# microscopic-image-analysis/DiffPointRasterisation.jl

Measured on AMD Instinct MI355X. Metric: M points/s fwd+bwd, 10M pts→256³ grid; HBM GB/s vs roofline, higher is better.
Workload: dtype f32

## Files before the change

### diffpointrasterisation.jl_amd/csrc/dpr_tiled.hip

```cpp
#include <hip/hip_runtime.h>

#include <cstring>
#include <mutex>
#include <set>
#include <type_traits>
#include <utility>

#include "dpr_tiled_impl.h"

namespace dpr {

template <int NO>
__device__ __forceinline__ int primary_tile(const int (&ref0)[NO], const TileGeom<NO>& tg) {
    int t = 0, stride = 1;
    bool in = true;
#pragma unroll
    for (int d = 0; d < NO; ++d) {
        const int r = ref0[d] < 0 ? 0 : ref0[d];
        int c = r / TileDims<NO>::T[d];
        if (d == NO - 1) {
            c -= tg.tz0;
            in = (unsigned)c < (unsigned)tg.nt[d];
        }
        t += c * stride;
// ... 1133 lines not shown
        return;
    }
    char* const wsp = ws + (size_t)blockIdx.y * pose_stride;
    const RunDesc* __restrict__ desc = (const RunDesc*)(wsp + off_desc);
    const uint32_t* __restrict__ blk_ndesc = (const uint32_t*)(wsp + off_bdesc);
    const uint32_t* __restrict__ tile_dstart = (const uint32_t*)(wsp + off_dstart);
    uint32_t* __restrict__ tile_cursor = (uint32_t*)(wsp + off_dcursor);
    RunDesc* __restrict__ sorted = (RunDesc*)(wsp + off_sdesc);
    const int lane = threadIdx.x & (kWave - 1), wave = threadIdx.x / kWave;
    if (fused) {
        const uint32_t* __restrict__ tile_ndesc = (const uint32_t*)(wsp + ra.off_ltot);
        const int NT = ra.NT;
        uint32_t c[4], sum = 0;
#pragma unroll
        for (int q = 0; q < 4; ++q) {
            const int i = threadIdx.x * 4 + q;
            c[q] = i < NT ? tile_ndesc[i] : 0u;
            sum += c[q];
        }
        uint32_t incl = sum;
#pragma unroll
        for (int o = 1; o < kWave; o <<= 1) {
            const uint32_t v = __shfl_up(incl, o, kWave);
            if (lane >= o) incl += v;
        }
        if (lane == kWave - 1) wsum[wave] = incl;
        __syncthreads();
        uint32_t run = incl - sum;
        for (int wv = 0; wv < wave; ++wv) run += wsum[wv];
#pragma unroll
        for (int q = 0; q < 4; ++q) {
            const int i = threadIdx.x * 4 + q;
            if (i < NT) s_dstart[i] = run;
            run += c[q];
        }
        __syncthreads();
    }
    const unsigned nblocks = fused ? gridDim.x - 1 : gridDim.x;
    const int64_t wave0 = (int64_t)blockIdx.x * (1024 / kWave) + wave;
    const int64_t nwaves = (int64_t)nblocks * (1024 / kWave);
    for (int64_t sub = wave0; sub < nsub; sub += nwaves) {
        const uint32_t n = blk_ndesc[sub] < (uint32_t)S ? blk_ndesc[sub] : (uint32_t)S;
        for (uint32_t i = lane; i < n; i += kWave) {
            const RunDesc d = desc[(size_t)sub * S + i];
            const uint32_t base = fused ? s_dstart[d.tile()] : tile_dstart[d.tile()];
            sorted[base + atomicAdd(&tile_cursor[d.tile()], 1u)] = d;
        }
    }
}

template <bool FIX, typename T, int NI, int NO, bool HAS_PW, typename R>
__device__ __forceinline__ void splat_record(const R& rc, bool active, const Pose<T, NI, NO>& ps,
                                             const GridDesc<NO>& gd, const int (&x0)[NO],
                                             double* __restrict__ acc, const FixScale& fs) {
    T pt[NI];
#pragma unroll
    for (int j = 0; j < NI; ++j) pt[j] = rc.v[j];
    const T w = HAS_PW ? ps.ow * rc.v[HAS_PW ? 3 : 0] : ps.ow * T(1);
    int ref0[NO];
    T dlo[NO];
    ref_and_deltas<T, NI, NO>(pt, ps, gd, ref0, dlo);
    int lb[NO];
    bool low_ok[NO];
#pragma unroll
    for (int d = 0; d < NO; ++d) {
        lb[d] = ref0[d] - x0[d];
        lb[d] = lb[d] < -1 ? -1 : (lb[d] > TileDims<NO>::T[d] - 1 ? TileDims<NO>::T[d] - 1 : lb[d]);
        low_ok[d] = lb[d] >= 0;
    }
    bool interior = true;
#pragma unroll
    for (int d = 0; d < NO; ++d) interior = interior && low_ok[d];
    if (active && interior) {
        double* base = &acc[lds_index<NO>(lb)];
#pragma unroll
        for (int s = 0; s < (1 << NO); ++s)
            cell_add<FIX, T>(base + nbr_lds_offset<NO>(s), voxel_weight<T, NO>(dlo, s, w), fs);
    } else if (active) {
#pragma unroll
        for (int s = 0; s < (1 << NO); ++s) {
            int l[NO];
            bool ok = true;
#pragma unroll
            for (int d = 0; d < NO; ++d) {
                const int sd = (s >> d) & 1;
                ok = ok && (sd || low_ok[d]);
                l[d] = (sd || low_ok[d]) ? lb[d] + sd : 0;
            }
            const T v = voxel_weight<T, NO>(dlo, s, w);
            cell_add<FIX, T>(&acc[lds_index<NO>(l)], ok ? v : T(0), fs);
        }
    }
}

template <bool FIX, typename T, int NI, int NO, typename R>
__device__ __forceinline__ void splat_record_jvp(const R& rc, const Rec4<T>& cf, bool active,
                                                 const Pose<T, NI, NO>& ps, const GridDesc<NO>& gd,
                                                 const int (&x0)[NO], double* __restrict__ acc, const FixScale& fs) {
    T pt[NI];
#pragma unroll
    for (int j = 0; j < NI; ++j) pt[j] = rc.v[j];
    int ref0[NO];
    T dlo[NO];
    ref_and_deltas<T, NI, NO>(pt, ps, gd, ref0, dlo);
    T bc[NO];
#pragma unroll
    for (int n = 0; n < NO; ++n) bc[n] = cf.v[1 + n];
    int lb[NO];
    bool low_ok[NO];
#pragma unroll
    for (int d = 0; d < NO; ++d) {
        lb[d] = ref0[d] - x0[d];
        lb[d] = lb[d] < -1 ? -1 : (lb[d] > TileDims<NO>::T[d] - 1 ? TileDims<NO>::T[d] - 1 : lb[d]);
        low_ok[d] = lb[d] >= 0;
    }
    bool interior = true;
#pragma unroll
    for (int d = 0; d < NO; ++d) interior = interior && low_ok[d];
    if (active && interior) {
        double* base = &acc[lds_index<NO>(lb)];
#pragma unroll
        for (int s = 0; s < (1 << NO); ++s)
            cell_add<FIX, T>(base + nbr_lds_offset<NO>(s), jvp_deposit<T, NO>(cf.v[0], bc, dlo, s), fs);
    } else if (active) {
#pragma unroll
        for (int s = 0; s < (1 << NO); ++s) {
            int l[NO];
            bool ok = true;
#pragma unroll
            for (int d = 0; d < NO; ++d) {
                const int sd = (s >> d) & 1;
                ok = ok && (sd || low_ok[d]);
                l[d] = (sd || low_ok[d]) ? lb[d] + sd : 0;
            }
            const T v = jvp_deposit<T, NO>(cf.v[0], bc, dlo, s);
            cell_add<FIX, T>(&acc[lds_index<NO>(l)], ok ? v : T(0), fs);
        }
    }
}

template <typename T, int NO>
__device__ __forceinline__ void flush_tile(const double* __restrict__ acc, const FixScale& fs, double bgv,
                                           const GridDesc<NO>& gd, const int (&x0)[NO], bool ghost_tile,
                                           T* __restrict__ o, T* __restrict__ hb) {
    constexpr int NVH = tile_voxels_halo<NO>();
    constexpr int TX = TileDims<NO>::T[0], TY = TileDims<NO>::T[1];
    constexpr int TZ = (NO == 3) ? TileDims<NO>::T[NO - 1] : 0;
    constexpr int ROWS = NVH / (TX + 1);
    constexpr int RPW = kWave / TX;
    static_assert(kWave % TX == 0, "tile rows must divide the wavefront");
    constexpr int NW = kSplatThreads / kWave;
    constexpr int kFB = 4;
    const int lane = threadIdx.x & (kWave - 1);
    const int x = lane % TX;
    const bool x_ok = x0[0] + x < gd.n[0];
    for (int row0 = (threadIdx.x / kWave) * RPW; row0 < ROWS; row0 += NW * RPW * kFB) {
        double raw[kFB];
        int rows[kFB];
#pragma unroll
        for (int u = 0; u < kFB; ++u) {
            int row = row0 + u * NW * RPW + lane / TX;
            if (RPW == 1) row = __builtin_amdgcn_readfirstlane(row);
            rows[u] = row;
            raw[u] = acc[(row < ROWS ? row : 0) * (TX + 1) + x];
        }
#pragma unroll
        for (int u = 0; u < kFB; ++u) {
            const int row = rows[u];
            if (row >= ROWS) continue;
            const int l1 = row % (TY + 1), l2 = (NO == 3) ? row / (TY + 1) : 0;
            const double a = fix_value(raw[u], fs);
            const bool owned = l1 < TY && (NO == 2 || l2 < TZ);
            if (owned) {
                const int g1 = x0[1] + l1, g2 = (NO == 3) ? x0[NO - 1] + l2 : 0;
                const bool in = g1 < gd.n[1] && (NO == 2 || g2 < gd.n[NO - 1]);
                if (in && x_ok && !ghost_tile)
                    __builtin_nontemporal_store(
                        (T)(bgv + a),
                        &o[((NO == 3) ? (size_t)g2 * gd.n[1] + g1 : (size_t)g1) * gd.n[0] + x0[0] + x]);
            } else {
                int h[NO];
                h[0] = x;
                h[1] = l1;
                if (NO == 3) h[NO - 1] = l2;
                hb[halo_index<NO>(h)] = (T)a;
            }
        }
    }
    for (int row = threadIdx.x; row < ROWS; row += kSplatThreads)
        hb[row] = (T)fix_value(acc[row * (TX + 1) + TX], fs);
}

template <typename T, int NI, int NO, bool HAS_PW, bool W3, bool WPL = false, bool JVP = false>
__global__ __launch_bounds__(kSplatThreads) void k_tile_splat(
    GridDesc<NO> gd, TileGeom<NO> tg, const RecT<T, W3>* __restrict__ rec,
    const WorkItem* __restrict__ items, const uint32_t* __restrict__ n_items,
    const uint32_t* __restrict__ tile_slab, const T* __restrict__ rot,
    const T* __restrict__ trans, const T* __restrict__ ow, const T* __restrict__ bg, int64_t b0,
    T* __restrict__ out, T* __restrict__ halo, T* __restrict__ ovf, int blocked,
    const uint32_t* __restrict__ maxpw, int fixed, const T* __restrict__ wplane) {
    static_assert(!WPL || (HAS_PW && !W3), "weight planes go with 4-word records and point weights");
    static_assert(!JVP || (HAS_PW && !W3 && !WPL), "coefficient records go with 4-word records");
    constexpr int NVH = tile_voxels_halo<NO>();
    __shared__ double acc[NVH];
    const uint32_t n_it = *n_items;
    const uint32_t order_flag = n_items[1];
    const float maxw_call = sizeof(T) == 4 ? guarded_max_weight(1.f, maxpw, HAS_PW) : __builtin_inff();
    const WorkItem item = items[blockIdx.x];
    Pose<T, NI, NO> ps = load_pose<T, NI, NO>(rot, trans, ow, b0);
    for (int i = threadIdx.x; i < NVH; i += kSplatThreads) acc[i] = 0.0;
    if (blockIdx.x >= n_it) return;
    if (blocked == 2) blocked = (NI == NO) ? (int)order_flag : 0;
    const int tile = (int)(item.tile % (uint32_t)tg.NT);
    const int64_t b = b0 + (int64_t)(item.tile / (uint32_t)tg.NT);
    int x0[NO], tc[NO];
    tile_origin<NO>(tile, tg, x0, tc);
    if (b != b0) ps = load_pose<T, NI, NO>(rot, trans, ow, b);
    uint32_t r1 = item.end;
    uint32_t r = item.begin;
    uint32_t step = kSplatThreads;
    if (blocked) {
        const uint32_t per = (r1 - r + kSplatThreads - 1) / kSplatThreads;
        r += threadIdx.x * per;
        r1 = (r + per < r1) ? r + per : r1;
        step = 1;
    } else {
        r += threadIdx.x;
    }
    constexpr int kPF = 2;
    RecT<T, W3> nxt[kPF];
    T nxt_w[WPL ? kPF : 1];
    Rec4<T> nxt_c[JVP ? kPF : 1];
    const Rec4<T>* const coef = (const Rec4<T>*)wplane;
#pragma unroll
    for (int u = 0; u < kPF; ++u) {
        const uint32_t ru = r + u * step;
        const uint32_t rl = ru < r1 ? ru : (r1 > item.begin ? r1 - 1 : item.begin);
        nxt[u] = rec[rl];
        if constexpr (WPL) nxt_w[u] = wplane[rl];
        if constexpr (JVP) nxt_c[u] = coef[rl];
    }
    lds_barrier();
    const FixScale fs = fix_scale(sizeof(T) == 4 ? fabsf((float)ps.ow) * maxw_call : __builtin_inff(),
                                  item.end - item.begin, fixed);
    auto record_loop = [&](auto fix_tag) {
        constexpr bool FIX = decltype(fix_tag)::value;
        while (r < r1) {
            RecT<T, W3> cur[kPF];
#pragma unroll
            for (int u = 0; u < kPF; ++u) cur[u] = nxt[u];
            if constexpr (WPL) {
#pragma unroll
                for (int u = 0; u < kPF; ++u) cur[u].v[3] = nxt_w[u];
            }
            Rec4<T> cur_c[JVP ? kPF : 1];
            if constexpr (JVP) {
#pragma unroll
                for (int u = 0; u < kPF; ++u) cur_c[u] = nxt_c[u];
            }
            const uint32_t r_cur = r;
            r += kPF * step;
#pragma unroll
            for (int u = 0; u < kPF; ++u) {
                const uint32_t ru = r + u * step;
                nxt[u] = rec[ru < r1 ? ru : r1 - 1];
                if constexpr (WPL) nxt_w[u] = wplane[ru < r1 ? ru : r1 - 1];
                if constexpr (JVP) nxt_c[u] = coef[ru < r1 ? ru : r1 - 1];
            }
#pragma unroll
            for (int u = 0; u < kPF; ++u) {
                if constexpr (JVP)
                    splat_record_jvp<FIX, T, NI, NO>(cur[u], cur_c[u], r_cur + u * step < r1, ps, gd, x0, acc, fs);
                else
                    splat_record<FIX, T, NI, NO, HAS_PW>(cur[u], r_cur + u * step < r1, ps, gd, x0, acc, fs);
            }
        }
    };
    if (fs.mul != 0.0) record_loop(std::true_type{});
    else record_loop(std::false_type{});
    lds_barrier();
    if ((item.part_nparts >> 16) > 1) {
        T* slab = ovf + (size_t)(tile_slab[item.tile] + (item.part_nparts & 0xffffu)) * NVH;
        constexpr int kSB = 4;
        for (int i0 = threadIdx.x; i0 < NVH; i0 += kSplatThreads * kSB) {
            double raw[kSB];
#pragma unroll
            for (int u = 0; u < kSB; ++u) {
                const int i = i0 + u * kSplatThreads;
                raw[u] = acc[i < NVH ? i : NVH - 1];
            }
#pragma unroll
            for (int u = 0; u < kSB; ++u) {
                const int i = i0 + u * kSplatThreads;
                if (i < NVH) slab[i] = (T)fix_value(raw[u], fs);
            }
        }
        return;
    }
    const double bgv = bg ? (double)bg[b] : 0.0;
    flush_tile<T, NO>(acc, fs, bgv, gd, x0, tg.ghost && tc[NO - 1] == 0 ,
                      out + b * gd.G, halo + (size_t)item.tile * halo_count<NO>());
}

template <typename T, int NI, int NO, bool HAS_PW, bool W3, bool RUNS>
__global__ __launch_bounds__(kSplatThreads, kSplatRunsOcc) void k_tile_splat_runs(
    GridDesc<NO> gd, TileGeom<NO> tg, const RecT<T, W3>* __restrict__ rec,
    const RunDesc* __restrict__ runs, uint32_t max_rec,
    const WorkItem* __restrict__ items, const uint32_t* __restrict__ n_items,
    const uint32_t* __restrict__ tile_slab, const T* __restrict__ rot,
    const T* __restrict__ trans, const T* __restrict__ ow, const T* __restrict__ bg, int64_t b0,
    T* __restrict__ out, T* __restrict__ halo, T* __restrict__ ovf, int blocked,
    const uint32_t* __restrict__ maxpw, int fixed) {
    constexpr int NVH = tile_voxels_halo<NO>();
    __shared__ double acc[NVH];
    const uint32_t n_it = *n_items;
    const WorkItem item = items[blockIdx.x];
    const float maxw_call = sizeof(T) == 4 ? guarded_max_weight(1.f, maxpw, HAS_PW) : __builtin_inff();
    Pose<T, NI, NO> ps = load_pose<T, NI, NO>(rot, trans, ow, b0);
    for (int i = threadIdx.x; i < NVH; i += kSplatThreads) acc[i] = 0.0;
    if (blockIdx.x >= n_it) return;
    const int tile = (int)(item.tile % (uint32_t)tg.NT);
    const int64_t b = b0 + (int64_t)(item.tile / (uint32_t)tg.NT);
    int x0[NO], tc[NO];
    tile_origin<NO>(tile, tg, x0, tc);
    if (b != b0) ps = load_pose<T, NI, NO>(rot, trans, ow, b);
    constexpr int kPF = 2;
    uint32_t n_bound = (item.end - item.begin) < (1u << 19) ? (item.end - item.begin) * 4096u : max_rec;
    n_bound = n_bound < max_rec ? n_bound : max_rec;
    const FixScale fs = fix_scale(sizeof(T) == 4 ? fabsf((float)ps.ow) * maxw_call : __builtin_inff(), n_bound, fixed);
    {
        __shared__ RunTable<kMaxRuns> rt;
        for (uint32_t d0 = item.begin; d0 < item.end; d0 += kMaxRuns) {
            const uint32_t d1 = (d0 + kMaxRuns < item.end) ? d0 + kMaxRuns : item.end;
            const int nruns = (int)(d1 - d0);
            const uint32_t n = load_runs(rt, runs, d0, d1, max_rec);
            const uint32_t per = (n + kSplatThreads - 1) / kSplatThreads;
            const uint32_t step = blocked ? 1u : (uint32_t)kSplatThreads;
            uint32_t i = blocked ? threadIdx.x * per : threadIdx.x;
            const uint32_t i1 = blocked ? ((i + per < n) ? i + per : n) : n;
            if (i < i1) {
                RunCursor cu;
                cu.seek(rt, i, nruns);
                uint32_t fetched = i;
                RecT<T, W3> nxt[kPF];
#pragma unroll
                for (int u = 0; u < kPF; ++u) {
                    const bool adv = fetched + step < i1;
                    nxt[u] = rec[cu.next(rt, adv ? step : 0u, nruns, adv)];
                    fetched += adv ? step : 0u;
                }
                while (i < i1) {
                    RecT<T, W3> cur[kPF];
#pragma unroll
                    for (int u = 0; u < kPF; ++u) cur[u] = nxt[u];
                    const uint32_t i_cur = i;
                    i += kPF * step;
#pragma unroll
                    for (int u = 0; u < kPF; ++u) {
                        const bool adv = fetched + step < i1;
                        nxt[u] = rec[cu.next(rt, adv ? step : 0u, nruns, adv)];
                        fetched += adv ? step : 0u;
                    }
#pragma unroll
                    for (int u = 0; u < kPF; ++u) {
                        if (fs.mul != 0.0)
                            splat_record<true, T, NI, NO, HAS_PW>(cur[u], i_cur + u * step < i1, ps, gd, x0, acc, fs);
                        else
                            splat_record<false, T, NI, NO, HAS_PW>(cur[u], i_cur + u * step < i1, ps, gd, x0, acc, fs);
                    }
                }
            }
            __syncthreads();
        }
    }
    lds_barrier();
    if ((item.part_nparts >> 16) > 1) {
        T* slab = ovf + (size_t)(tile_slab[item.tile] + (item.part_nparts & 0xffffu)) * NVH;
        constexpr int kSB = 4;
        for (int i0 = threadIdx.x; i0 < NVH; i0 += kSplatThreads * kSB) {
            double raw[kSB];
#pragma unroll
            for (int u = 0; u < kSB; ++u) {
                const int i = i0 + u * kSplatThreads;
                raw[u] = acc[i < NVH ? i : NVH - 1];
            }
#pragma unroll
            for (int u = 0; u < kSB; ++u) {
                const int i = i0 + u * kSplatThreads;
                if (i < NVH) slab[i] = (T)fix_value(raw[u], fs);
            }
        }
        return;
    }
    const double bgv = bg ? (double)bg[b] : 0.0;
    flush_tile<T, NO>(acc, fs, bgv, gd, x0, tg.ghost && tc[NO - 1] == 0 ,
                      out + b * gd.G, halo + (size_t)item.tile * halo_count<NO>());
}

template <int NO> __host__ __device__ constexpr int low_face_count() {
    if (NO == 2) return TileDims<2>::T[0] + TileDims<2>::T[1] - 1;
    return TileDims<3>::T[0] * TileDims<3>::T[1] + TileDims<3>::T[0] * (TileDims<3>::T[2] - 1) +
           (TileDims<3>::T[1] - 1) * (TileDims<3>::T[2] - 1);
}
template <int NO> __device__ __forceinline__ void low_face_coords(int i, int (&l)[NO]) {
    constexpr int TX = TileDims<NO>::T[0], TY = TileDims<NO>::T[1];
    if constexpr (NO == 2) {
        if (i < TX) {
            l[0] = i;
            l[1] = 0;
        } else {
            l[0] = 0;
            l[1] = 1 + (i - TX);
        }
    } else {
        constexpr int TZ = TileDims<NO>::T[2];
        if (i < TX * TY) {
            l[0] = i % TX;
            l[1] = i / TX;
            l[2] = 0;
        } else if (i < TX * TY + TX * (TZ - 1)) {
            const int j = i - TX * TY;
            l[0] = j % TX;
            l[1] = 0;
            l[2] = 1 + j / TX;
        } else {
            const int j = i - TX * TY - TX * (TZ - 1);
            l[0] = 0;
            l[1] = 1 + j % (TY - 1);
            l[2] = 1 + j / (TY - 1);
        }
    }
}

template <typename T, int NO>
__device__ __forceinline__ void halo_gather_tile(const GridDesc<NO>& gd, const TileGeom<NO>& tg,
                                                 const T* __restrict__ halo,
                                                 const T* __restrict__ ovf,
                                                 const uint32_t* __restrict__ tile_parts,
                                                 const uint32_t* __restrict__ tile_slab,
                                                 const T* __restrict__ bg, int64_t b0,
                                                 T* __restrict__ out, bool any_split, int ptile,
                                                 bool split, int c) {
    constexpr int NV = tile_voxels<NO>();
    constexpr int NVH = tile_voxels_halo<NO>();
    constexpr int CH = kSplitChunks;
    const int i_begin = split ? c * 256 : 0;
    const int i_end = split ? NV : low_face_count<NO>();
    const int tile = ptile % tg.NT;
    const int pbase = ptile - tile;
    const int64_t b = b0 + ptile / tg.NT;
    const int i_step = split ? 256 * CH : 256;
    int x0[NO], tc[NO];
    tile_origin<NO>(tile, tg, x0, tc);
    if (tg.ghost && tc[NO - 1] == 0) return;
    T* o = out + b * gd.G;
    constexpr int NC = 1 << NO;
    uint32_t nparts[NC], nslab[NC];
    bool nvalid[NC], any_nbr_split = false;
    int nsrc[NC];
#pragma unroll
    for (int m = 1; m < NC; ++m) {
        bool v = true;
        int src = ptile, tstride = 1;
#pragma unroll
        for (int d = 0; d < NO; ++d) {
            if ((m >> d) & 1) {
                v = v && tc[d] > 0;
                src -= tstride;
            }
            tstride *= tg.nt[d];
        }
        nvalid[m] = v;
        nsrc[m] = v ? src : ptile;
        nparts[m] = any_split ? tile_parts[nsrc[m]] : 1u;
        nslab[m] = any_split ? tile_slab[nsrc[m]] : 0u;
        any_nbr_split = any_nbr_split || (v && nparts[m] > 1);
    }
    if constexpr (NO == 3 && TileDims<NO>::T[0] == kWave) {
        if (split) {
            constexpr int TX = TileDims<NO>::T[0], TY = TileDims<NO>::T[1], TZ = TileDims<NO>::T[2];
            constexpr int YF = (TY + 1) * (TZ + 1), ZF = YF + TX * (TZ + 1);
            constexpr int NW = 256 / kWave, RIT = kSplitRows / NW;
            static_assert(kSplitRows % NW == 0 && (TY * TZ) % kSplitRows == 0, "whole rows per wave");
            static_assert(kSplitChunks * kSplitRows == TY * TZ, "chunks cover the tile");
            const int lane = threadIdx.x & (kWave - 1), wave = threadIdx.x / kWave;
            const uint32_t my_parts = tile_parts[ptile], my_slab = tile_slab[ptile];
            const double bgv = bg ? (double)bg[b] : 0.0;
            const bool x_ok = x0[0] + lane < gd.n[0];
            const size_t HC = halo_count<NO>();
            double own[RIT];
            bool act[RIT];
            int offs[RIT], cell[RIT], l1s[RIT], l2s[RIT];
#pragma unroll
            for (int k = 0; k < RIT; ++k) {
                const int row = __builtin_amdgcn_readfirstlane(c * kSplitRows + wave * RIT + k);
                l1s[k] = row % TY;
                l2s[k] = row / TY;
                const int g1 = x0[1] + l1s[k], g2 = x0[2] + l2s[k];
                act[k] = x_ok && g1 < gd.n[1] && g2 < gd.n[2];
                offs[k] = act[k] ? (g2 * gd.n[1] + g1) * gd.n[0] + x0[0] + lane : 0;
                cell[k] = lane + (TX + 1) * (l1s[k] + (TY + 1) * l2s[k]);
                own[k] = bgv;
            }
            const T* sp = ovf + (size_t)my_slab * NVH;
            for (uint32_t q = 0; q < my_parts; ++q) {
                T a[RIT];
#pragma unroll
                for (int k = 0; k < RIT; ++k) a[k] = sp[(size_t)q * NVH + cell[k]];
#pragma unroll
                for (int k = 0; k < RIT; ++k) own[k] += (double)a[k];
            }
            auto nbr = [&](int m, bool on, int hidx, int ncell) -> double {
                if (nparts[m] > 1) {
                    const T* np_ = ovf + (size_t)nslab[m] * NVH + (on ? ncell : 0);
                    double sum = 0.0;
                    for (uint32_t q = 0; q < nparts[m]; ++q) sum += (double)np_[(size_t)q * NVH];
                    return on ? sum : 0.0;
                }
                const T v = halo[on ? (size_t)nsrc[m] * HC + hidx : (size_t)0];
                return on ? (double)v : 0.0;
            };
#pragma unroll
            for (int k = 0; k < RIT; ++k) {
                const int l1 = l1s[k], l2 = l2s[k];
                const bool lowy = l1 == 0, lowz = l2 == 0, l0z = lane == 0;
                if (!(lowy || lowz || nvalid[1])) {
                    if (act[k]) o[offs[k]] = (T)own[k];
                    continue;
                }
                double add = 0.0;
                if (nvalid[1]) add += nbr(1, act[k] && l0z, l1 + (TY + 1) * l2, TX + (TX + 1) * (l1 + (TY + 1) * l2));
                if (lowy && nvalid[2]) add += nbr(2, act[k], YF + lane + TX * l2, lane + (TX + 1) * (TY + (TY + 1) * l2));
                if (lowy && nvalid[3]) add += nbr(3, act[k] && l0z, TY + (TY + 1) * l2, TX + (TX + 1) * (TY + (TY + 1) * l2));
                if (lowz && nvalid[4]) add += nbr(4, act[k], ZF + lane + TX * l1, lane + (TX + 1) * (l1 + (TY + 1) * TZ));
                if (lowz && nvalid[5]) add += nbr(5, act[k] && l0z, l1 + (TY + 1) * TZ, TX + (TX + 1) * (l1 + (TY + 1) * TZ));
                if (lowy && lowz && nvalid[6])
                    add += nbr(6, act[k], YF + TX * TZ + lane, lane + (TX + 1) * (TY + (TY + 1) * TZ));
                if (lowy && lowz && nvalid[7])
                    add += nbr(7, act[k] && l0z, TY + (TY + 1) * TZ, TX + (TX + 1) * (TY + (TY + 1) * TZ));
                if (act[k]) o[offs[k]] = (T)(own[k] + add);
            }
            return;
        }
        if (!split) {
            constexpr int TX = TileDims<NO>::T[0], TY = TileDims<NO>::T[1], TZ = TileDims<NO>::T[2];
            constexpr int NROW = TY + TZ - 1, NW = 256 / kWave, RIT = (NROW + NW - 1) / NW;
            constexpr int YF = (TY + 1) * (TZ + 1), ZF = YF + TX * (TZ + 1);
            static_assert(TY * TZ <= 256, "one thread per l0 == 0 voxel");
            const int lane = threadIdx.x & (kWave - 1), wave = threadIdx.x / kWave;
            const bool x_ok = x0[0] + lane < gd.n[0] && lane >= 1;
            const T* hy_t = halo + (size_t)nsrc[2] * halo_count<NO>() + YF + lane;
            const T* hz_t = halo + (size_t)nsrc[4] * halo_count<NO>() + ZF + lane;
            const T* hyz_t = halo + (size_t)nsrc[6] * halo_count<NO>() + YF + TX * TZ + lane;
            const bool uy = nvalid[2] && nparts[2] == 1, uz = nvalid[4] && nparts[4] == 1,
                       uyz = nvalid[6] && nparts[6] == 1;
            T cur[RIT], vy[RIT], vz[RIT], vyz[RIT];
            bool act[RIT], by[RIT], bz[RIT];
            int offs[RIT];
#pragma unroll
            for (int k = 0; k < RIT; ++k) {
                const int row = __builtin_amdgcn_readfirstlane(wave + k * NW);
                const bool live = row < NROW;
                const int l1 = row < TY ? row : 0, l2 = row < TY ? 0 : row - (TY - 1);
                const int g1 = x0[1] + l1, g2 = x0[2] + l2;
                by[k] = live && l1 == 0 && tc[1] > 0;
                bz[k] = live && l2 == 0 && tc[2] > 0;
                act[k] = live && x_ok && g1 < gd.n[1] && g2 < gd.n[2] && (by[k] || bz[k]);
                offs[k] = act[k] ? (g2 * gd.n[1] + g1) * gd.n[0] + x0[0] + lane : 0;
                cur[k] = o[offs[k]];
                vy[k] = *((act[k] && by[k] && uy) ? hy_t + TX * l2 : halo);
                vz[k] = *((act[k] && bz[k] && uz) ? hz_t + TX * l1 : halo);
                vyz[k] = *((act[k] && by[k] && bz[k] && uyz) ? hyz_t : halo);
            }
            const int j = threadIdx.x < TY * TZ ? threadIdx.x : 0;
            const int lB[NO] = {0, j % TY, j / TY};
            int offB = 0, strideB = 1;
            bool okB = threadIdx.x < TY * TZ, lowB = false;
#pragma unroll
            for (int d = 0; d < NO; ++d) {
                const int gcoord = x0[d] + lB[d];
                okB = okB && gcoord < gd.n[d];
                lowB = lowB || (lB[d] == 0 && tc[d] > 0);
                offB += gcoord * strideB;
                strideB *= gd.n[d];
            }
            const bool actB = okB && lowB;
            offB = actB ? offB : 0;
            const T curB = o[offB];
            T vB[8];
            bool bB[8];
            int cellB[8];
#pragma unroll
            for (int m = 1; m < 8; ++m) {
                bool valid = actB && nvalid[m];
                int h[NO];
#pragma unroll
                for (int d = 0; d < NO; ++d) {
                    const bool in_m = (m >> d) & 1;
                    valid = valid && (!in_m || lB[d] == 0);
                    h[d] = in_m ? TileDims<NO>::T[d] : lB[d];
                }
                bB[m] = valid;
                cellB[m] = lds_index<NO>(h);
                const size_t hi = (valid && nparts[m] == 1)
                                      ? (size_t)nsrc[m] * halo_count<NO>() + halo_index<NO>(h)
                                      : (size_t)0;
                vB[m] = halo[hi];
            }
            double addA[RIT][3], addB[8];
#pragma unroll
            for (int k = 0; k < RIT; ++k) {
                addA[k][0] = (act[k] && by[k] && uy) ? (double)vy[k] : 0.0;
                addA[k][1] = (act[k] && bz[k] && uz) ? (double)vz[k] : 0.0;
                addA[k][2] = (act[k] && by[k] && bz[k] && uyz) ? (double)vyz[k] : 0.0;
            }
#pragma unroll
            for (int m = 1; m < 8; ++m) addB[m] = (bB[m] && nparts[m] == 1) ? (double)vB[m] : 0.0;
            if (any_nbr_split) {
                auto slab_sum = [&](int m, int cell) {
                    const T* sp = ovf + (size_t)nslab[m] * NVH + cell;
                    double sum = 0.0;
                    uint32_t q = 0;
                    for (; q + 4 <= nparts[m]; q += 4) {
                        const T a0 = sp[(size_t)q * NVH], a1 = sp[(size_t)(q + 1) * NVH],
                                a2 = sp[(size_t)(q + 2) * NVH], a3 = sp[(size_t)(q + 3) * NVH];
                        sum += (double)a0;
                        sum += (double)a1;
                        sum += (double)a2;
                        sum += (double)a3;
                    }
                    for (; q < nparts[m]; ++q) sum += (double)sp[(size_t)q * NVH];
                    return sum;
                };
#pragma unroll
                for (int k = 0; k < RIT; ++k) {
                    const int row = __builtin_amdgcn_readfirstlane(wave + k * NW);
                    const int l1 = row < TY ? row : 0, l2 = row < TY ? 0 : row - (TY - 1);
                    if (nvalid[2] && nparts[2] > 1 && act[k] && by[k])
                        addA[k][0] = slab_sum(2, lane + (TX + 1) * (TY + (TY + 1) * l2));
                    if (nvalid[4] && nparts[4] > 1 && act[k] && bz[k])
                        addA[k][1] = slab_sum(4, lane + (TX + 1) * (l1 + (TY + 1) * TZ));
                    if (nvalid[6] && nparts[6] > 1 && act[k] && by[k] && bz[k])
                        addA[k][2] = slab_sum(6, lane + (TX + 1) * (TY + (TY + 1) * TZ));
                }
#pragma unroll
                for (int m = 1; m < 8; ++m)
                    if (bB[m] && nparts[m] > 1) addB[m] = slab_sum(m, cellB[m]);
            }
#pragma unroll
            for (int k = 0; k < RIT; ++k) {
                const double add = (addA[k][0] + addA[k][1]) + addA[k][2];
                if (act[k]) o[offs[k]] = (T)((double)cur[k] + add);
            }
            double sumB = 0.0;
#pragma unroll
            for (int m = 1; m < 8; ++m) sumB += addB[m];
            if (actB) o[offB] = (T)((double)curB + sumB);
            return;
        }
    }
    if (!any_split) {
        constexpr int IT = (low_face_count<NO>() + 255) / 256;
        T cur[IT];
        double add[IT];
        int offs[IT];
        bool act[IT];
#pragma unroll
        for (int k = 0; k < IT; ++k) {
            const int i = threadIdx.x + k * 256;
            int l[NO];
            low_face_coords<NO>(i < low_face_count<NO>() ? i : 0, l);
            int off = 0, stride = 1;
            bool ok = i < low_face_count<NO>(), low = false;
#pragma unroll
            for (int d = 0; d < NO; ++d) {
                const int gcoord = x0[d] + l[d];
                ok = ok && gcoord < gd.n[d];
// ... 1490 lines not shown
```

### diffpointrasterisation.jl_amd/csrc/dpr_tiled_impl.h

```cpp
#pragma once
#include <hip/hip_runtime.h>

#include "../../include/dpr.h"
#include "dpr_device.h"
#include "dpr_jvp.h"
#include "dpr_tiled.h"

namespace dpr {

template <int NO> struct TileDims;
template <> struct TileDims<3> {
    static constexpr int T[3] = {64, 16, 8};
};
template <> struct TileDims<2> {
    static constexpr int T[3] = {32, 32, 1};
};
constexpr int kMaxTiles = 32768;
constexpr int kBinThreads = 1024;
constexpr int kWcThreads = 1024;
constexpr int kWcPpt = 4;
constexpr int kSplatThreads = 512;
constexpr int kSplatRunsOcc = 4;
template <typename T> __host__ __device__ constexpr int gather_threads() {
    return sizeof(T) == 8 ? 512 : 256;
}
template <typename T> __host__ __device__ constexpr int gather_waves_per_simd() { return 4; }
constexpr int kUpb = 4;
constexpr int kGatherRb = 8;
constexpr int kMaxBinBlocks = 512;
constexpr int kSplitChunks = 8;
constexpr int kSplitRows = 16;
constexpr int kSplitGrid = 2048;

template <int NO> struct TileGeom {
    int nt[NO];
    int NT;
    int tz0;
    int ghost;
};

template <int NO> __host__ __device__ constexpr int tile_voxels() {
    int v = 1;
    for (int d = 0; d < NO; ++d) v *= TileDims<NO>::T[d];
    return v;
}
template <int NO> __host__ __device__ constexpr int tile_voxels_halo() {
    int v = 1;
    for (int d = 0; d < NO; ++d) v *= TileDims<NO>::T[d] + 1;
    return v;
}
template <int NO> __host__ __device__ constexpr int halo_count() {
    return tile_voxels_halo<NO>() - tile_voxels<NO>();
}

struct SlabCut {
    int per_layer, layers, lps, nslab;
};

constexpr uint32_t kBinMagic = 0x44505242u, kBinValid = 1u;
struct alignas(16) BinHeader {
    uint32_t magic, state;
    uint32_t elem, n_in, n_out, has_pw;
    int64_t P;
    int32_t grid[3];
    uint32_t verdict;
    uint64_t points, pw;
    uint32_t layout, pad_[3];
    unsigned char pose[96];
};

struct alignas(16) WorkItem {
    uint32_t tile, begin, end;
    uint32_t part_nparts;
};

struct alignas(8) RunDesc {
    uint32_t start;
    uint32_t tile_count;
    __host__ __device__ uint32_t tile() const { return tile_count & 0x7fffu; }
    __host__ __device__ uint32_t count() const { return tile_count >> 15; }
};
constexpr int kMaxLocalTiles = 16384;
constexpr int kMaxRuns = 256;
constexpr int kMaxRunsGather = 64;

struct Plan {
    int bg;
    int nblk;
    int64_t chunk;
    uint32_t cap;
    int max_items;
    int max_slabs;
    size_t off_hdr, off_counts, off_totals, off_tile_start, off_items, off_nitems, off_nzbins, off_tparts, off_tslab,
        off_split, off_rec, off_idx, off_slot, off_aux, total;
    bool sort_inside;
    size_t off_spts, off_spw, off_perm, off_iperm, off_sgrad, off_sgradw, off_sorttmp;
    size_t pose_stride;
    bool local;
    int lb;
    int64_t copies;
    int sub;
    int64_t nsub;
    int64_t max_desc;
    size_t off_ltot, off_dstart, off_dcursor, off_bdesc, off_desc, off_sdesc;
};

template <int NO> bool make_slab_cut(const int64_t* grid, SlabCut* sc);
template <int NO> TileGeom<NO> slab_geom(const int64_t* grid, const SlabCut& sc, int s, bool forward);
int slab_max_tiles(const SlabCut& sc);

struct PlanRequest {
    size_t elem;
    int n_in, n_out;
    int tiles;
    int64_t P, B;
    int max_group;
    bool coherent;
    bool share_batch;
    bool slabbed;
    bool fwd_only;
};
PlanRequest plan_request(size_t elem, int op, unsigned flags, int n_in, int n_out, const SlabCut& sc, int64_t P,
                         int64_t B);
Plan make_plan(const PlanRequest& rq);
Plan pose_plan(size_t elem, int n_in, int n_out, const SlabCut& sc, int64_t P);
uint32_t plan_layout_id(const Plan& pl);
int tiled_check(int n_out, const int64_t* grid, int64_t P, unsigned flags, const char* binning_flag, SlabCut* sc);
bool pose_binning_cut(int n_out, const int64_t* grid, int64_t P, SlabCut* sc);
size_t channel_part_bytes(size_t elem, int64_t P, int C);
size_t jvp_part_bytes(size_t elem, int64_t P);

size_t coarse_workspace_bytes(size_t elem, int64_t P);

}
```

Baseline: 27120.

## Distribute splat runs to waves dynamically via LDS atomic counter

Replaces the block-wide shared run table, where all 512 threads cursor through a chunk of up to 256 runs and then synchronise, with per-wave work stealing. Each wave takes whole runs from an LDS atomic counter, splits a run's records across its lanes, and prefetches the next run descriptor while splatting. This removes the run-table loads, the cursor seeking and the per-chunk __syncthreads. In exchange, waves become imbalanced when runs are very uneven in length, and lanes go idle on short runs.

```diff
diff --git a/diffpointrasterisation.jl_amd/csrc/dpr_tiled.hip b/diffpointrasterisation.jl_amd/csrc/dpr_tiled.hip
--- a/diffpointrasterisation.jl_amd/csrc/dpr_tiled.hip
+++ b/diffpointrasterisation.jl_amd/csrc/dpr_tiled.hip
@@ -1459,6 +1459,18 @@
                       out + b * gd.G, halo + (size_t)item.tile * halo_count<NO>());
 }
 
+__device__ __forceinline__ RunDesc wave_run_desc(const RunDesc* __restrict__ runs, uint32_t k,
+                                                 const WorkItem& item) {
+    RunDesc d{0u, 0u};
+    if (item.begin < item.end) d = runs[k < item.end ? k : item.end - 1];
+    return d;
+}
+__device__ __forceinline__ uint32_t draw_run(uint32_t* next_run) {
+    uint32_t v = 0;
+    if ((threadIdx.x & (kWave - 1)) == 0) v = atomicAdd(next_run, 1u);
+    return __builtin_amdgcn_readfirstlane(v);
+}
+
 template <typename T, int NI, int NO, bool HAS_PW, bool W3, bool RUNS>
 __global__ __launch_bounds__(kSplatThreads, kSplatRunsOcc) void k_tile_splat_runs(
     GridDesc<NO> gd, TileGeom<NO> tg, const RecT<T, W3>* __restrict__ rec,
@@ -1469,13 +1481,18 @@
     T* __restrict__ out, T* __restrict__ halo, T* __restrict__ ovf, int blocked,
     const uint32_t* __restrict__ maxpw, int fixed) {
     constexpr int NVH = tile_voxels_halo<NO>();
+    constexpr uint32_t NW = kSplatThreads / kWave;
     __shared__ double acc[NVH];
+    __shared__ uint32_t next_run;
     const uint32_t n_it = *n_items;
     const WorkItem item = items[blockIdx.x];
     const float maxw_call = sizeof(T) == 4 ? guarded_max_weight(1.f, maxpw, HAS_PW) : __builtin_inff();
     Pose<T, NI, NO> ps = load_pose<T, NI, NO>(rot, trans, ow, b0);
+    if (blockIdx.x >= n_it) return;
+    uint32_t k = item.begin + (uint32_t)__builtin_amdgcn_readfirstlane(threadIdx.x / kWave);
+    RunDesc d = wave_run_desc(runs, k, item);
     for (int i = threadIdx.x; i < NVH; i += kSplatThreads) acc[i] = 0.0;
-    if (blockIdx.x >= n_it) return;
+    if (threadIdx.x == 0) next_run = NW;
     const int tile = (int)(item.tile % (uint32_t)tg.NT);
     const int64_t b = b0 + (int64_t)(item.tile / (uint32_t)tg.NT);
     int x0[NO], tc[NO];
@@ -1485,51 +1502,49 @@
     uint32_t n_bound = (item.end - item.begin) < (1u << 19) ? (item.end - item.begin) * 4096u : max_rec;
     n_bound = n_bound < max_rec ? n_bound : max_rec;
     const FixScale fs = fix_scale(sizeof(T) == 4 ? fabsf((float)ps.ow) * maxw_call : __builtin_inff(), n_bound, fixed);
-    {
-        __shared__ RunTable<kMaxRuns> rt;
-        for (uint32_t d0 = item.begin; d0 < item.end; d0 += kMaxRuns) {
-            const uint32_t d1 = (d0 + kMaxRuns < item.end) ? d0 + kMaxRuns : item.end;
-            const int nruns = (int)(d1 - d0);
-            const uint32_t n = load_runs(rt, runs, d0, d1, max_rec);
-            const uint32_t per = (n + kSplatThreads - 1) / kSplatThreads;
-            const uint32_t step = blocked ? 1u : (uint32_t)kSplatThreads;
-            uint32_t i = blocked ? threadIdx.x * per : threadIdx.x;
-            const uint32_t i1 = blocked ? ((i + per < n) ? i + per : n) : n;
-            if (i < i1) {
-                RunCursor cu;
-                cu.seek(rt, i, nruns);
-                uint32_t fetched = i;
-                RecT<T, W3> nxt[kPF];
+    lds_barrier();
+    auto walk_runs = [&](auto fix_tag) {
+        constexpr bool FIX = decltype(fix_tag)::value;
+        const uint32_t lane = threadIdx.x & (kWave - 1);
+        while (k < item.end) {
+            const uint32_t st = d.start < max_rec ? d.start : max_rec;
+            const uint32_t c = d.count() < max_rec - st ? d.count() : max_rec - st;
+            const RecT<T, W3>* __restrict__ const rr = rec + st;
+            const uint32_t per = (c + kWave - 1) / kWave;
+            const uint32_t step = blocked ? 1u : (uint32_t)kWave;
+            uint32_t o = blocked ? lane * per : lane;
+            const uint32_t o1 = blocked ? (o + per < c ? o + per : c) : c;
+            RecT<T, W3> nxt[kPF];
+            if (c) {
 #pragma unroll
                 for (int u = 0; u < kPF; ++u) {
-                    const bool adv = fetched + step < i1;
-                    nxt[u] = rec[cu.next(rt, adv ? step : 0u, nruns, adv)];
-                    fetched += adv ? step : 0u;
+                    const uint32_t ou = o + u * step;
+                    nxt[u] = rr[ou < o1 ? ou : o1 - 1];
                 }
-                while (i < i1) {
-                    RecT<T, W3> cur[kPF];
-#pragma unroll
-                    for (int u = 0; u < kPF; ++u) cur[u] = nxt[u];
-                    const uint32_t i_cur = i;
-                    i += kPF * step;
-#pragma unroll
-                    for (int u = 0; u < kPF; ++u) {
-                        const bool adv = fetched + step < i1;
-                        nxt[u] = rec[cu.next(rt, adv ? step : 0u, nruns, adv)];
-                        fetched += adv ? step : 0u;
-                    }
-#pragma unroll
-                    for (int u = 0; u < kPF; ++u) {
-                        if (fs.mul != 0.0)
-                            splat_record<true, T, NI, NO, HAS_PW>(cur[u], i_cur + u * step < i1, ps, gd, x0, acc, fs);
-                        else
-                            splat_record<false, T, NI, NO, HAS_PW>(cur[u], i_cur + u * step < i1, ps, gd, x0, acc, fs);
-                    }
+            }
+            const uint32_t kn = item.begin + draw_run(&next_run);
+            const RunDesc dn = wave_run_desc(runs, kn, item);
+            while (o < o1) {
+                RecT<T, W3> cur[kPF];
+#pragma unroll
+                for (int u = 0; u < kPF; ++u) cur[u] = nxt[u];
+                const uint32_t o_cur = o;
+                o += kPF * step;
+#pragma unroll
+                for (int u = 0; u < kPF; ++u) {
+                    const uint32_t ou = o + u * step;
+                    nxt[u] = rr[ou < o1 ? ou : o1 - 1];
                 }
-            }
-            __syncthreads();
-        }
-    }
+#pragma unroll
+                for (int u = 0; u < kPF; ++u)
+                    splat_record<FIX, T, NI, NO, HAS_PW>(cur[u], o_cur + u * step < o1, ps, gd, x0, acc, fs);
+            }
+            k = kn;
+            d = dn;
+        }
+    };
+    if (fs.mul != 0.0) walk_runs(std::true_type{});
+    else walk_runs(std::false_type{});
     lds_barrier();
     if ((item.part_nparts >> 16) > 1) {
         T* slab = ovf + (size_t)(tile_slab[item.tile] + (item.part_nparts & 0xffffu)) * NVH;
diff --git a/diffpointrasterisation.jl_amd/csrc/dpr_tiled_impl.h b/diffpointrasterisation.jl_amd/csrc/dpr_tiled_impl.h
--- a/diffpointrasterisation.jl_amd/csrc/dpr_tiled_impl.h
+++ b/diffpointrasterisation.jl_amd/csrc/dpr_tiled_impl.h
@@ -81,7 +81,6 @@
     __host__ __device__ uint32_t count() const { return tile_count >> 15; }
 };
 constexpr int kMaxLocalTiles = 16384;
-constexpr int kMaxRuns = 256;
 constexpr int kMaxRunsGather = 64;
 
 struct Plan {
```

Measured after the change: 27200, median of 6. Within noise of the previous version (+0.3%).
